# zyrlia1018/CMD-GEN

Measured on AMD Instinct MI355X. Metric: denoising steps/sec, higher is better.
Workload: dtype f32

## Files before the change

### cmdgen_amd/csrc/cmdgen_api.hip

```cpp
#include "cmdgen_host.h"
#include "cmdgen_launch.h"
#include "cmdgen_wlayout.h"

std::string g_create_error;

extern "C" const char* cmdgen_version(void) { return "cmdgen_hip 0.1 (gfx950)"; }

extern "C" const char* cmdgen_last_error(const cmdgen_handle* h) { return h ? h->err.c_str() : g_create_error.c_str(); }

extern "C" int cmdgen_create(const cmdgen_config* cfg, int device, cmdgen_handle** out) {
    if (!cfg || !out) return fail(nullptr, CMDGEN_EINVAL, "null argument");
    const int H = cfg->hidden_nf;
    if (!(H == 64 || H == 128 || H == 256 || H == 512))
        return fail(nullptr, CMDGEN_EINVAL, "hidden_nf=%d unsupported: the gfx950 kernels tile 64 columns per wave and are built for 64, 128, 256 and 512", H);
    if (cfg->inv_sublayers < 1 || cfg->inv_sublayers > 8) return fail(nullptr, CMDGEN_EINVAL, "inv_sublayers=%d out of range [1, 8]", cfg->inv_sublayers);
    if (cfg->n_layers < 1 || cfg->n_layers > CMDGEN_MAX_LAYERS) return fail(nullptr, CMDGEN_EINVAL, "n_layers out of range");
    if (cfg->phar_nf < 1 || 2 * cfg->phar_nf > CMDGEN_MAX_SMALL || cfg->residue_nf < 1 ||
        2 * cfg->residue_nf > CMDGEN_MAX_SMALL || cfg->joint_nf < 1 || cfg->joint_nf + 1 > CMDGEN_MAX_SMALL)
        return fail(nullptr, CMDGEN_EINVAL, "feature sizes exceed the small-MLP bound %d", CMDGEN_MAX_SMALL);
    if (cfg->timesteps < 1) return fail(nullptr, CMDGEN_EINVAL, "timesteps < 1");
    if (cfg->update_pocket_coords && cfg->no_com_projection)
        return fail(nullptr, CMDGEN_EINVAL, "update_pocket_coords (joint model) and no_com_projection (SimpleConditionalDDPM) are exclusive");
    int ndev = 0;
    if (hipGetDeviceCount(&ndev) != hipSuccess || device < 0 || device >= ndev)
// ... 140 lines not shown
    GET(dy + "phar_encoder.0.weight", 2 * d.P * d.P); UP(s.pe0_w); GET(dy + "phar_encoder.0.bias", 2 * d.P); UP(s.pe0_b);
    GET(dy + "phar_encoder.2.weight", d.J * 2 * d.P); UP(s.pe2_w); GET(dy + "phar_encoder.2.bias", d.J); UP(s.pe2_b);
    GET(dy + "phar_decoder.0.weight", 2 * d.P * d.J); UP(s.pd0_w); GET(dy + "phar_decoder.0.bias", 2 * d.P); UP(s.pd0_b);
    GET(dy + "phar_decoder.2.weight", d.P * 2 * d.P); UP(s.pd2_w); GET(dy + "phar_decoder.2.bias", d.P); UP(s.pd2_b);
    GET(dy + "residue_encoder.0.weight", 2 * d.R * d.R); UP(s.re0_w); GET(dy + "residue_encoder.0.bias", 2 * d.R); UP(s.re0_b);
    GET(dy + "residue_encoder.2.weight", d.J * 2 * d.R); UP(s.re2_w); GET(dy + "residue_encoder.2.bias", d.J); UP(s.re2_b);
    GET(dy + "residue_decoder.0.weight", 2 * d.R * d.J); UP(s.rd0_w); GET(dy + "residue_decoder.0.bias", 2 * d.R); UP(s.rd0_b);
    GET(dy + "residue_decoder.2.weight", d.R * 2 * d.R); UP(s.rd2_w); GET(dy + "residue_decoder.2.bias", d.R); UP(s.rd2_b);
    {
        std::vector<float> pack;
        for (const char* nm : {"phar_encoder.0.weight", "phar_encoder.0.bias", "phar_encoder.2.weight", "phar_encoder.2.bias",
                               "residue_encoder.0.weight", "residue_encoder.0.bias", "residue_encoder.2.weight", "residue_encoder.2.bias"}) {
            auto it = h->staged.find(dy + nm);
            if (it == h->staged.end()) return fail(h, CMDGEN_ESTATE, "missing tensor '%s%s'", dy.c_str(), nm);
            pack.insert(pack.end(), it->second.begin(), it->second.end());
        }
        rc = upload(h, pack, &s.enc_pack); if (rc) return rc;
    }
    {
        GET(dy + "egnn.embedding.weight", H * d.dyn);
        std::vector<float> t((size_t)H * d.dyn);
        for (int c = 0; c < H; ++c) for (int k = 0; k < d.dyn; ++k) t[(size_t)k * H + c] = (*v)[(size_t)c * d.dyn + k];
        rc = upload(h, t, &s.emb_wT); if (rc) return rc;
        GET(dy + "egnn.embedding.bias", H); UP(s.emb_b);
    }
    {
        GET(dy + "egnn.embedding_out.weight", d.dyn * H);
        std::vector<float> t((size_t)H * d.dyn);
        for (int j = 0; j < d.dyn; ++j) for (int k = 0; k < H; ++k) t[(size_t)k * d.dyn + j] = (*v)[(size_t)j * H + k];
        rc = upload(h, t, &s.embo_wT); if (rc) return rc;
        GET(dy + "egnn.embedding_out.bias", d.dyn); UP(s.embo_b);
    }
    const int nfeat = d.sin ? 24 : 2;
    const int ld1 = 2 * H + nfeat;
    for (int b = 0; b < d.L; ++b)
    for (int sub = 0; sub < d.S; ++sub) {
        LayerW lw{};
        const std::string g = dy + "egnn.e_block_" + std::to_string(b) + ".gcl_" + std::to_string(sub) + ".";
        const std::string c = dy + "egnn.e_block_" + std::to_string(b) + ".gcl_equiv.";
        auto split_first = [&](const std::string& wname, const std::string& bname, WPack* Wpq,
                               const float** bias, const float** wr, const float** wd, const float** we) -> int {
            const std::vector<float>* w; int r = get_w(h, wname, (size_t)H * ld1, &w); if (r) return r;
            std::vector<float> AB((size_t)2 * H * H);
            std::vector<float> vr(H), vd(H);
            for (int o = 0; o < H; ++o) {
                for (int k = 0; k < H; ++k) {
// ... 41 lines not shown
#undef GET
#undef UP
    h->layers = std::move(layers);
    h->finalized = true;
    h->user_coef_K = -1;
    release_chains(h);
    if (h->have_layout) replan(h);
    return CMDGEN_OK;
}

static inline size_t edge_lds_bytes(int max_n) { return (size_t)max_n * (sizeof(float4) + 3 * sizeof(int)); }
static const size_t kEdgeLdsMax = 156 * 1024;

PlanInput plan_input(const cmdgen_handle* h) {
    PlanInput in;
    const Dims& d = h->dims;
    in.H = d.H; in.L = d.L; in.S = d.S; in.joint = d.joint != 0; in.sin = d.sin != 0; in.cutoff = d.cutoff2 >= 0.f;
    in.n_cus = h->n_cus; in.gemm_split = h->gemm_split;
    in.B = (int)h->cur_nphar.size(); in.nph = h->cur_nphar.data(); in.npk = h->cur_npocket.data();
    in.N = h->lay.N; in.Nl = h->lay.Nl; in.max_n = h->lay.max_n;
    in.opts = &h->opts;
    if (!h->layers.empty()) {
        in.W2 = in.W7 = in.Wpq_e = PlanPacks::of_uploaded(d.H); in.W3 = PlanPacks::of_uploaded(2 * d.H);
    }
    return in;
}
void replan(cmdgen_handle* h) { h->plan = make_plan(plan_input(h)); }

static int set_layout_impl(cmdgen_handle* h, int64_t batch, const int64_t* nph, const int64_t* npk, bool on_stream, hipStream_t stream);
extern "C" int cmdgen_set_layout(cmdgen_handle* h, int64_t batch, const int64_t* nph, const int64_t* npk) {
    return set_layout_impl(h, batch, nph, npk, false, nullptr);
}
extern "C" int cmdgen_set_layout_on_stream(cmdgen_handle* h, int64_t batch, const int64_t* nph, const int64_t* npk, cmdgen_stream stream) {
    return set_layout_impl(h, batch, nph, npk, true, (hipStream_t)stream);
}
static int set_layout_impl(cmdgen_handle* h, int64_t batch, const int64_t* nph, const int64_t* npk, bool on_stream, hipStream_t stream) {
    if (!h || batch < 1 || !nph || !npk) return fail(h, CMDGEN_EINVAL, "bad layout arguments");
    if (h->have_layout && (int64_t)h->cur_nphar.size() == batch &&
        memcmp(h->cur_nphar.data(), nph, batch * sizeof(int64_t)) == 0 &&
        memcmp(h->cur_npocket.data(), npk, batch * sizeof(int64_t)) == 0)
        return CMDGEN_OK;
    ++h->eval_gen;
    hipSetDevice(h->device);
    const Dims& d = h->dims;
    const int B = (int)batch;
    std::vector<int> vph(B), vpk(B), bph(B), bpk(B);
// ... 117 lines not shown
    if (!h) return CMDGEN_EINVAL;
    if (!h->have_layout) return fail(h, CMDGEN_ESTATE, "no batch layout (cmdgen_set_layout)");
    hipSetDevice(h->device);
    h->last_stream = s;
    if (h->agg_dirty) {
        HIPCHK(h, hipMemsetAsync(h->work.agg, 0, (size_t)h->lay.N * h->dims.H * sizeof(float), s));
        h->agg_dirty = false;
    }
    return 0;
}

EvalLaunch make_launch(cmdgen_handle* h) {
    EvalLaunch a; a.lay = h->lay; a.w = h->work; a.d = h->dims; a.sw = h->small; a.layers = h->layers.data();
    a.plan = h->plan;
    a.prof_events = nullptr; a.ablate = 0;
    if (!a.plan.node64 && !a.plan.dead_skip) a.w.need_qc = nullptr;
    a.w.hop_levels = a.plan.dead_skip >= 2 ? h->dims.L : 1;
    if (!a.plan.dead_skip) a.w.ehop = nullptr;
    return a;
}

static const char* const kOptionKeys[] = {
    "node_mt", "edge_mt", "coord_mt", "embed_mt", "edge_wgs_per_cu", "coord_wgs_per_cu", "e128_wgs_per_cu", "e128_fused", "half_engine", "edge_fullk", "node64", "node16_split", "node16w",
    "proj_in_coord", "dead_skip", "write_embed", "graph_steps",
    "wgrad_split", "wgrad_tile", "wgrad_split_wgs128", "wgrad_split_wgs64", "wgrad_wgs", "dgrad_mt", "dgrad_tail", "wgrad_stream", "train_half", "wgrad_silu", "train_node16", "wgrad_k128"};

static void drop_graphs(cmdgen_handle* h) {
    hipSetDevice(h->device);
    if (h->own_stream) hipStreamSynchronize(h->own_stream);
    if (h->have_layout) hipStreamSynchronize(h->last_stream);
    drop_chain_graphs(h);
}
static void refresh_tune(cmdgen_handle* h) {
    TrainTune t;
    t.wgrad_split = (int)opt_of(h, "wgrad_split", t.wgrad_split); t.wgrad_tile = (int)opt_of(h, "wgrad_tile", t.wgrad_tile);
    t.wgrad_split_wgs128 = (int)opt_of(h, "wgrad_split_wgs128", t.wgrad_split_wgs128); t.wgrad_split_wgs64 = (int)opt_of(h, "wgrad_split_wgs64", t.wgrad_split_wgs64);
    t.wgrad_wgs = (int)opt_of(h, "wgrad_wgs", t.wgrad_wgs); t.dgrad_mt = (int)opt_of(h, "dgrad_mt", t.dgrad_mt); t.dgrad_tail = (int)opt_of(h, "dgrad_tail", t.dgrad_tail);
    t.wgrad_stream = (int)opt_of(h, "wgrad_stream", t.wgrad_stream); t.wgrad_k128 = (int)opt_of(h, "wgrad_k128", t.wgrad_k128);
    h->tune = t;
}

extern "C" int cmdgen_set_option(cmdgen_handle* h, const char* key, int64_t value, int32_t unset) {
    if (!h || !key) return fail(h, CMDGEN_EINVAL, "null argument");
    bool known = false;
    for (const char* k : kOptionKeys) known = known || strcmp(k, key) == 0;
    if (!known) return fail(h, CMDGEN_EINVAL, "unknown option '%s'", key);
    drop_graphs(h);
// ... 891 lines not shown
```

### cmdgen_amd/csrc/cmdgen_dev.h

```cpp
#pragma once
#include <hip/hip_runtime.h>
#include <stdint.h>
#include <vector>
#include "cmdgen_split.h"
#include "cmdgen_plan.h"

typedef float f32x16 __attribute__((ext_vector_type(16)));

#define CMDGEN_MAX_LAYERS 16
#define CMDGEN_MAX_SMALL 64

struct WPack {
    const float4* w32;
    const float4* w16;
    const void*   ws;
    const void*   ws16;
    const void*   wh;
    const void*   wh16;
    float         wh_scale;
    float         wh_inv;
    const float*  wh_dev;
};

struct LayerW {
// ... 8 lines not shown
    const float*  ba;
    WPack W3;
    const float*  b3;
    WPack W4;
    const float*  b4;
    WPack Wpq_c;
    const float*  b6;
    const float*  wr_c;
    const float*  wd_c;
    const float*  we_c;
    WPack W7;
    const float*  b7;
    const float*  w5;
};

struct SmallW {
    const float *pe0_w, *pe0_b, *pe2_w, *pe2_b;
    const float *pd0_w, *pd0_b, *pd2_w, *pd2_b;
    const float *re0_w, *re0_b, *re2_w, *re2_b;
    const float *rd0_w, *rd0_b, *rd2_w, *rd2_b;
    const float *emb_wT, *emb_b;
    const float *embo_wT, *embo_b;
    const float *enc_pack;
};

struct Dims {
    int P, R, J, H, L;
    int dyn;
    int attention, use_tanh, condition_time;
    int no_com;
    int joint;
    float cutoff2;
    float norm_constant, norm_factor, coords_range;
    int S;
    int sin;
    float sin_freq[6];
    int agg_mean;
    float norm_x, norm_h, bias_h;
};

struct Layout {
    int B, Nl, Np, N;
    int Nm;
    int max_n;
    const int* num_phar;
    const int* num_pocket;
    const int* phar_base;
// ... 406 lines not shown
```

### cmdgen_amd/csrc/cmdgen_plan.h

```cpp
#pragma once
#include <cstdint>
#include <cstring>
#include <map>
#include <string>

enum class PlanEngine { fp32, bf3, half };
inline int plan_mfmas_per_product(PlanEngine e) { return e == PlanEngine::fp32 ? 1 : e == PlanEngine::bf3 ? 6 : 3; }

enum class MsgKernel { tiles, fullk32, e128 };
enum class NodeKernel { tiles, node16w, node32p, node64, node64e, node64d };
enum class CoordKernel { tiles, fullk32, fullk32_proj, e128 };

struct PlanPacks {
    bool ws = false, wh = false, ws16 = false, wh16 = false;
    static PlanPacks of_uploaded(int in) { return PlanPacks{true, true, in % 128 == 0, in % 128 == 0}; }
};

struct PlanInput {
    int H = 256, L = 1, S = 1;
    bool joint = false, sin = false, cutoff = true;
    int n_cus = 256;
    bool gemm_split = true;
    int B = 0;
    const int64_t* nph = nullptr; const int64_t* npk = nullptr;
    int N = 0, Nl = 0, max_n = 0;
    const std::map<std::string, int64_t>* opts = nullptr;
    PlanPacks W2, W3, W7, Wpq_e;
    bool training = false;
    int E = 0, Ec = 0;

    int64_t opt(const char* key, int64_t dflt) const { if (!opts) return dflt; auto it = opts->find(key); return it == opts->end() ? dflt : it->second; }
    bool opt_set(const char* key) const { return opts && opts->find(key) != opts->end(); }
};

struct LaunchPlan {
    MsgKernel msg = MsgKernel::tiles; NodeKernel node = NodeKernel::tiles; CoordKernel coord = CoordKernel::tiles;
    PlanEngine msg_eng = PlanEngine::fp32, node_eng = PlanEngine::fp32, coord_eng = PlanEngine::fp32;
    int node_mt = 64, edge_mt = 64, coord_mt = 64;
    int embed_mt = 16;
    int edge_grid = 512, coord_grid = 256, e128_grid = 512;
    int e128_fused = 3;
    int dead_skip = 0, write_embed = 1;
    int gemm_split = 1, half_engine = 0, node16_split = 0, node64 = 0, node16w = 1, edge_fullk = 0, proj_in_coord = 0;
    bool fwd_half = false, node_half = false;
    bool reads_frag = false;
};

inline LaunchPlan make_plan(const PlanInput& in) {
    LaunchPlan p;
    const int n_cus = in.n_cus, H = in.H;
    const bool split = in.gemm_split, sp256 = H == 256 && split;
    const int he_opt = (int)in.opt("half_engine", 1);
    const bool half_opt = he_opt == 2 || (he_opt == 1 && in.cutoff);
    const bool half = sp256 && half_opt;
    p.gemm_split = split ? 1 : 0;
    p.half_engine = split && half_opt ? 1 : 0;

    double e_est = 0.0, ec_est = 0.0;
    const int64_t N = (int64_t)in.N;
    for (int b = 0; b < in.B; ++b) {
        const double n = (double)(in.nph[b] + in.npk[b]);
        const bool full = !in.cutoff;
        const double deg = full ? n : (n <= 128.0 ? 9.0 : 36.0);
        const double dnode = deg < n ? deg : n;
        double dphar = full ? n : 0.6 * (double)in.nph[b] + (n <= 128.0 ? 0.15 : 0.13) * (double)in.npk[b];
        if (dphar > n) dphar = n;
// ... 45 lines not shown
    {
        int on = 0;
        if (sp256 && n_cus > 0) {
            const int ncu = n_cus, t64 = (in.N + 63) / 64, t32 = (in.N + 31) / 32;
            const float cost64 = (float)((t64 + ncu - 1) / ncu);
            const int full = t32 / (2 * ncu), rem = t32 - full * 2 * ncu;
            float cost32 = 1.12f * full + (rem == 0 ? 0.f : rem <= ncu ? 0.62f : 1.12f);
            if (half) cost32 = 1.9f * full + (rem == 0 ? 0.f : rem <= ncu ? 1.22f : 1.9f);
            on = cost64 < cost32 && !(half && node_mt == 16);
            if (half && node_mt != 16) on = 32;
            if (on == 32 && t32 > ncu && t64 <= ncu) on = 8;
            else if (on == 32 && t64 > ncu) on = 2;
            if (in.opt_set("node64")) { const int64_t v = in.opt("node64", 0); on = v == 32 ? 32 : v == 8 ? 8 : v == 2 ? 2 : v != 0; }
        }
        p.node64 = on;
        p.dead_skip = (in.joint || in.S != 1) ? 0 : (int)in.opt("dead_skip", 2);
    }
    p.node16_split = (split && H >= 128 && in.opt("node16_split", 1) != 0) ? 1 : 0;
    p.node16w = in.opt("node16w", 1) != 0 ? 1 : 0;
    {
        p.embed_mt = (int)in.opt("embed_mt", (((double)in.Nl / 16.0 <= 2.0 * n_cus && !in.joint) ? 16 : node_mt));
        if (p.embed_mt != 16 && p.embed_mt != 32 && p.embed_mt != 64) p.embed_mt = node_mt;
    }
    if (split && node_mt == 64 && !in.opt_set("node_mt")) node_mt = 32;
    p.node_mt = node_mt; p.edge_mt = edge_mt; p.coord_mt = coord_mt;

    const PlanEngine tiles32 = split ? PlanEngine::bf3 : PlanEngine::fp32;
    if (in.training) {
        const int train_half = (int)in.opt("train_half", 1);
        p.fwd_half = sp256 && half_opt && p.edge_fullk && in.W2.wh && train_half != 0;
        if (p.fwd_half && in.opt("train_node16", 1) != 0) p.node_mt = 16;
        p.node_half = p.fwd_half && p.node_mt == 16 && in.W3.wh16 && train_half != 2;
        p.dead_skip = 0; p.node64 = 0; p.proj_in_coord = 0;
        auto rows = [&](int n) { return n / 64 >= 4 * n_cus ? 64 : (n / 32 >= n_cus / 4 ? 32 : 16); };
        auto grid = [&](int n, int mt) { const int cap = (mt >= 64 ? 2 : 4) * n_cus, g = (int)((n / mt + 1) * 1.25) + 8; return g < n_cus / 4 ? n_cus / 4 : (g > cap ? cap : g); };
        if (!in.opt_set("edge_mt") || p.edge_mt == 128) { p.edge_mt = rows(in.E); p.edge_grid = grid(in.E, p.edge_mt); }
        if (!in.opt_set("coord_mt") || p.coord_mt == 128) { p.coord_mt = rows(in.Ec); p.coord_grid = grid(in.Ec, p.coord_mt); }
        if (p.fwd_half) {
            p.edge_mt = 32; p.edge_grid = grid(in.E, 32); p.coord_mt = 32; p.coord_grid = grid(in.Ec, 32);
        }
        const PlanEngine save32 = split && H == 256 && in.W2.ws ? PlanEngine::bf3 : PlanEngine::fp32;
        p.msg = p.fwd_half ? MsgKernel::fullk32 : MsgKernel::tiles;
        p.msg_eng = p.fwd_half ? PlanEngine::half : (p.edge_mt >= 32 ? save32 : PlanEngine::fp32);
        p.coord = p.fwd_half ? CoordKernel::fullk32 : CoordKernel::tiles;
        p.coord_eng = p.fwd_half ? PlanEngine::half : (p.coord_mt >= 32 ? save32 : PlanEngine::fp32);
        p.node = p.node_half && H == 256 ? NodeKernel::node16w : NodeKernel::tiles;
// ... 11 lines not shown
        p.node = p.node64 == 2 && eight ? NodeKernel::node64d : p.node64 == 8 && eight ? NodeKernel::node64e : p.node64 == 32 ? NodeKernel::node32p : NodeKernel::node64;
    } else if (H == 256 && node_mt == 16 && p.node16_split && p.node16w && in.W3.ws16) {
        p.node = NodeKernel::node16w; p.node_eng = half && in.W3.wh16 ? PlanEngine::half : PlanEngine::bf3;
    } else {
        p.node = NodeKernel::tiles;
        p.node_eng = node_mt >= 32 ? tiles32 : (p.node16_split && in.W3.ws16 ? PlanEngine::bf3 : PlanEngine::fp32);
    }
    if (coord_mt == 128 && in.W7.ws) { p.coord = CoordKernel::e128; p.coord_eng = half && in.W7.wh ? PlanEngine::half : PlanEngine::bf3; }
    else if (p.edge_fullk && coord_mt == 32) { p.coord = CoordKernel::fullk32; p.coord_eng = half && in.W7.wh ? PlanEngine::half : PlanEngine::bf3; }
    else { p.coord = CoordKernel::tiles; p.coord_eng = coord_mt >= 32 ? tiles32 : PlanEngine::fp32; }
    p.reads_frag = p.msg == MsgKernel::tiles || p.coord == CoordKernel::tiles || p.node == NodeKernel::tiles;
    const bool can = p.node == NodeKernel::node16w && p.coord == CoordKernel::fullk32 && in.S == 1 && in.L > 1 && !in.joint && p.node_eng == p.coord_eng &&
                     (p.node_eng == PlanEngine::half ? in.Wpq_e.wh16 : in.Wpq_e.ws16);
    p.proj_in_coord = can && in.opt("proj_in_coord", 1) != 0 ? 1 : 0;
    if (p.proj_in_coord) p.coord = CoordKernel::fullk32_proj;
    return p;
}

inline bool plan_query(const LaunchPlan& p, const char* key, int64_t* value) {
    const struct { const char* key; int64_t v; } keys[] = {
        {"node_mt", p.node_mt}, {"edge_mt", p.edge_mt}, {"coord_mt", p.coord_mt}, {"edge_grid", p.edge_grid}, {"coord_grid", p.coord_grid},
        {"e128_fused", p.e128_fused}, {"gemm_split", p.gemm_split}, {"half_engine", p.half_engine}, {"node16_split", p.node16_split},
        {"node64", p.node64}, {"node16w", p.node16w}, {"proj_in_coord", p.proj_in_coord}, {"edge_fullk", p.edge_fullk}, {"dead_skip", p.dead_skip},
        {"msg_mfmas_per_product", plan_mfmas_per_product(p.msg_eng)}, {"node_mfmas_per_product", plan_mfmas_per_product(p.node_eng)},
        {"coord_mfmas_per_product", plan_mfmas_per_product(p.coord_eng)}};
    for (const auto& k : keys) if (strcmp(k.key, key) == 0) { *value = k.v; return true; }
    return false;
}
```

### cmdgen_amd/csrc/kernels_egnn_graph.hip

```cpp
#ifndef CMDGEN_H_PART
#define CMDGEN_H_PART 0
#endif
#include "cmdgen_egnn_common.h"

__device__ __forceinline__ int flat_node(int i, int nl, int pb, int qb, int Nl) {
    return i < nl ? pb + i : Nl + qb + (i - nl);
}

#if CMDGEN_H_PART == 0
__global__ void k_edge_count(Layout lay, Work w, Dims d, const float* __restrict__ xh_phar,
                             const float* __restrict__ xh_pocket) {
    extern __shared__ float4 spos[];
    int* sdeg = reinterpret_cast<int*>(spos + lay.max_n);
    const int b = blockIdx.x, tid = threadIdx.x;
    const int nl = lay.num_phar[b], np = lay.num_pocket[b], n = nl + np;
    const int pb = lay.phar_base[b], qb = lay.pocket_base[b];
    const int ldp = 3 + d.P, ldq = 3 + d.R;
    for (int i = tid; i < n; i += blockDim.x) {
        float4 p;
        if (i < nl) {
            const float* s = xh_phar + (size_t)(pb + i) * ldp;
            p = make_float4(s[0], s[1], s[2], 0.f);
            w.X0[pb + i] = p;
            for (int l = 0; l < d.L; ++l) w.ACC[(size_t)l * lay.Nm + pb + i] = make_float4(0.f, 0.f, 0.f, 0.f);
// ... 186 lines not shown
                for (int e = lane; e < dg; e += 64) w.ehop[off + e] = lvl;
            }
        }
    }
    if (b == 0 && tid == 0) *w.nan_flag = 0;
    if (b == lay.B - 1 && tid == 0) {
        const int E = s_base[1] + (w.pocketE[b] - eph_b);
        const int Ec = d.joint ? s_base[4] + w.pocketEnsQ[b] : s_base[3] + w.pocketEns[b];
        w.totals[0] = E; w.totals[1] = Ec;
        atomicAdd(&w.counters[1], (unsigned long long)E);
        atomicAdd(&w.counters[2], (unsigned long long)Ec);
    }
}
#if CMDGEN_H_PART == 0
__global__ void k_edge_write(Layout lay, Work w, Dims d) { edge_write_body(lay, w, d, blockIdx.x); }
#endif

template <int H, int MT, bool SP>
__device__ __forceinline__ void embed_body(const Layout& lay, const Work& w, const Dims& d, const SmallW& sw, const LayerW& lw0,
                                           const float* __restrict__ xh_phar,
                                           const float* __restrict__ xh_pocket,
                                           const float* __restrict__ t_arr,
                                           const float4* __restrict__ coef, const ChainState* chain, const TrainSave& sv,
                                           const PocketCache& pc, const int blk, const int part = 2) {
    if (pc.c != nullptr && blk * MT >= lay.Nl) {
        const int row0 = blk * MT, nvalid = min(MT, lay.N - row0);
        const float t = coef[chain->step].w;
        constexpr int LPR = H / 4;
        const int c4 = threadIdx.x % LPR, rsub = threadIdx.x / LPR;
        const float4 dh = reinterpret_cast<const float4*>(pc.dh)[c4], dP = reinterpret_cast<const float4*>(pc.dP)[c4],
                     dQ = reinterpret_cast<const float4*>(pc.dQ)[c4];
        auto axpy = [&](const float4& a, const float4& b) { return make_float4(fmaf(t, b.x, a.x), fmaf(t, b.y, a.y), fmaf(t, b.z, a.z), fmaf(t, b.w, a.w)); };
#pragma unroll 4
        for (int r = rsub; r < nvalid; r += 4) {
            const size_t q = (size_t)(row0 + r - lay.Nl) * LPR + c4, o = (size_t)(row0 + r) * LPR + c4;
            reinterpret_cast<float4*>(w.h)[o] = axpy(reinterpret_cast<const float4*>(pc.c)[q], dh);
            reinterpret_cast<float4*>(w.P)[o] = axpy(reinterpret_cast<const float4*>(pc.P0)[q], dP);
            reinterpret_cast<float4*>(w.Q)[o] = axpy(reinterpret_cast<const float4*>(pc.Q0)[q], dQ);
        }
        return;
    }
#if CMDGEN_STAMPS == 3
    unsigned long long est_[8] = {0,0,0,0,0,0,0,0}, est_t = __builtin_amdgcn_s_memtime(); const unsigned long long est_b = est_t;
#define ESTAMP(i) do { const unsigned long long n_ = __builtin_amdgcn_s_memtime(); est_[i] += n_ - est_t; est_t = n_; } while (0)
#else
#define ESTAMP(i) do {} while (0)
#endif
    __shared__ __attribute__((aligned(16))) float buf[MT * LDA(H)];
    __shared__ float s_in[MT][CMDGEN_MAX_SMALL];
    __shared__ float s_h1[MT][CMDGEN_MAX_SMALL];
    __shared__ float s_h2[MT][CMDGEN_MAX_SMALL + 1];
    const int tid = threadIdx.x, nthr = H;
    const int row0 = blk * MT;
    const int nvalid = min(MT, lay.N - row0);
    const int ldp = 3 + d.P, ldq = 3 + d.R;
    const int Fmax = max(d.P, d.R), F1max = 2 * Fmax;
    typedef Eng<MT, SP> G;
    typename G::Carry carry;
    const typename G::Frag f0 = G::frag(lw0.Wpq_e, H / 8, 0, (part == 1 ? H / 64 : 0) + (tid >> 6));
    G::prefetch(f0, carry);
    const ColVec<MT> b1v = col_load<MT>(lw0.b1, tid >> 6);
    const float t_chain = t_arr ? 0.f : coef[chain->step].w;
    extern __shared__ float s_enc[];
    const int seg_n[8] = {2 * d.P * d.P, 2 * d.P, d.J * 2 * d.P, d.J, 2 * d.R * d.R, 2 * d.R, d.J * 2 * d.R, d.J};
    const float* const seg_p[8] = {sw.pe0_w, sw.pe0_b, sw.pe2_w, sw.pe2_b, sw.re0_w, sw.re0_b, sw.re2_w, sw.re2_b};
    int seg_o[9];
    seg_o[0] = 0;
#pragma unroll
    for (int q = 0; q < 8; ++q) seg_o[q + 1] = seg_o[q] + seg_n[q];
    constexpr int NIN = (MT * CMDGEN_MAX_SMALL + H - 1) / H;
    float vin[NIN];
#pragma unroll
    for (int q = 0; q < NIN; ++q) {
        const int idx = tid + q * nthr;
        vin[q] = 0.f;
        if (idx < MT * Fmax) {
            const int r = idx / Fmax, k = idx - r * Fmax, n = row0 + r;
            if (r < nvalid) {
                if (n < lay.Nl) { if (k < d.P) vin[q] = xh_phar[(size_t)n * ldp + 3 + k]; }
                else if (k < d.R) vin[q] = xh_pocket[(size_t)(n - lay.Nl) * ldq + 3 + k];
            }
        }
    }
    if (sw.enc_pack) {
        for (int i = tid; i < seg_o[8]; i += nthr) s_enc[i] = sw.enc_pack[i];
    } else
    for (int base = 0; base < seg_o[8]; base += 16 * nthr) {
        float v[16];
#pragma unroll
        for (int q = 0; q < 16; ++q) {
            const int gi = base + q * nthr + tid;
            v[q] = 0.f;
            if (gi < seg_o[8]) {
                int sg = 0;
#pragma unroll
                for (int u = 1; u < 8; ++u) sg += gi >= seg_o[u];
                v[q] = seg_p[sg][gi - seg_o[sg]];
            }
        }
#pragma unroll
        for (int q = 0; q < 16; ++q) {
            const int gi = base + q * nthr + tid;
            if (gi < seg_o[8]) s_enc[gi] = v[q];
        }
    }
    const float *pe0w = s_enc + seg_o[0], *pe0b = s_enc + seg_o[1], *pe2w = s_enc + seg_o[2], *pe2b = s_enc + seg_o[3];
    const float *re0w = s_enc + seg_o[4], *re0b = s_enc + seg_o[5], *re2w = s_enc + seg_o[6], *re2b = s_enc + seg_o[7];
#pragma unroll
    for (int q = 0; q < NIN; ++q) {
        const int idx = tid + q * nthr;
        if (idx < MT * Fmax) { const int r = idx / Fmax; s_in[r][idx - r * Fmax] = vin[q]; }
    }
    lds_barrier();
    ESTAMP(0);
    for (int idx = tid; idx < MT * F1max; idx += nthr) {
        const int r = idx / F1max, o = idx - r * F1max;
        const int n = row0 + r;
        if (r >= nvalid) continue;
        const bool ph = n < lay.Nl;
        const int F = ph ? d.P : d.R;
        if (o >= 2 * F) continue;
        const float* W = (ph ? pe0w : re0w) + o * F;
        float s = (ph ? pe0b : re0b)[o];
#pragma unroll 4
        for (int k = 0; k < F; ++k) s = fmaf(s_in[r][k], W[k], s);
        const float act = silu_f(s);
        s_h1[r][o] = act;
        if (sv.enc1_l) {
            if (ph) { sv.enc1_l[(size_t)n * 2 * F + o] = s; sv.enca_l[(size_t)n * 2 * F + o] = act; }
            else { sv.enc1_p[(size_t)(n - lay.Nl) * 2 * F + o] = s; sv.enca_p[(size_t)(n - lay.Nl) * 2 * F + o] = act; }
        }
    }
    lds_barrier();
    ESTAMP(1);
    for (int idx = tid; idx < MT * d.dyn; idx += nthr) {
        const int r = idx / d.dyn, j = idx - r * d.dyn;
        const int n = row0 + r;
        float s = 0.f;
        if (r < nvalid) {
            if (j < d.J) {
                const bool ph = n < lay.Nl;
                const int F2 = 2 * (ph ? d.P : d.R);
                const float* W = (ph ? pe2w : re2w) + j * F2;
                s = (ph ? pe2b : re2b)[j];
#pragma unroll 4
                for (int k = 0; k < F2; ++k) s = fmaf(s_h1[r][k], W[k], s);
            } else {
                s = t_arr ? t_arr[lay.node_sample[n]] : t_chain;
            }
            if (sv.hdyn) sv.hdyn[(size_t)n * d.dyn + j] = s;
        }
        s_h2[r][j] = s;
    }
    lds_barrier();
    ESTAMP(2);
    {
        const int c = tid;
        const float bc = sw.emb_b[c];
        float accr[MT];
#pragma unroll
        for (int r = 0; r < MT; ++r) accr[r] = bc;
        for (int k0 = 0; k0 < d.dyn; k0 += 16) {
            float wk[16];
#pragma unroll
            for (int j = 0; j < 16; ++j) wk[j] = k0 + j < d.dyn ? sw.emb_wT[(size_t)(k0 + j) * H + c] : 0.f;
#pragma unroll
            for (int j = 0; j < 16; ++j)
                if (k0 + j < d.dyn) {
#pragma unroll
                    for (int r = 0; r < MT; ++r) accr[r] = fmaf(s_h2[r][k0 + j], wk[j], accr[r]);
                }
        }
#pragma unroll
        for (int r = 0; r < MT; ++r) {
            const float s = r < nvalid ? accr[r] : 0.f;
            buf[r * LDA(H) + c] = s;
            if (r < nvalid && part != 1) {
                w.h[(size_t)(row0 + r) * H + c] = s;
                if (sv.h) sv.h[(size_t)(row0 + r) * H + c] = s;
            }
        }
    }
    lds_barrier();
    ESTAMP(3);
    tile_project_pq<H, MT, SP>(buf, lw0.Wpq_e, b1v, w.P, w.Q, row0, nvalid, part != 1, carry, f0, part != 0);
    ESTAMP(4);
#if CMDGEN_STAMPS == 3
    if ((threadIdx.x & 63) == 0) { const int wv = threadIdx.x >> 6; for (int i = 0; i < 5; ++i) atomicAdd(&w.dbg[wv * 8 + i], est_[i]);
        atomicAdd(&w.dbg[32 + wv], __builtin_amdgcn_s_memtime() - est_b); atomicAdd(&w.dbg[40], 1ull); }
#endif
#undef ESTAMP
}
template <int H, int MT, bool SP>
__global__ __launch_bounds__(H) void k_embed(Layout lay, Work w, Dims d, SmallW sw, LayerW lw0, const float* __restrict__ xh_phar,
                                             const float* __restrict__ xh_pocket, const float* __restrict__ t_arr,
                                             const float4* __restrict__ coef, const ChainState* chain, TrainSave sv, PocketCache pc) {
    embed_body<H, MT, SP>(lay, w, d, sw, lw0, xh_phar, xh_pocket, t_arr, coef, chain, sv, pc, (int)blockIdx.x);
}
template <int MT, bool SP>
__global__ __launch_bounds__(256) void k_write_embed(Layout lay, Work w, Dims d, SmallW sw, LayerW lw0, const float* __restrict__ xh_phar,
                                                     const float* __restrict__ xh_pocket, const float* __restrict__ t_arr,
                                                     const float4* __restrict__ coef, const ChainState* chain, PocketCache pc, int npair) {
    const int i = (int)blockIdx.x - lay.B;
    if (i < 0) edge_write_body(lay, w, d, (int)blockIdx.x);
    else if (i < 2 * npair) embed_body<256, MT, SP>(lay, w, d, sw, lw0, xh_phar, xh_pocket, t_arr, coef, chain, TrainSave{}, pc, i >> 1, i & 1);
    else embed_body<256, MT, SP>(lay, w, d, sw, lw0, xh_phar, xh_pocket, t_arr, coef, chain, TrainSave{}, pc, i - npair, 2);
}

template <int H, int MT, bool SP> static void launch_embed(const EvalLaunch& a, const float* xp, const float* xq, const float* t,
                                                  const float4* coef, ChainState* chain, hipStream_t s) {
    if constexpr (H == 512 && MT == 64) launch_embed<H, 32, SP>(a, xp, xq, t, coef, chain, s);
    else {
        const int nt = (a.lay.N + MT - 1) / MT;
        const Dims& d = a.d;
        const size_t shm = sizeof(float) * (size_t)(2 * d.P * d.P + 2 * d.P + d.J * 2 * d.P + d.J + 2 * d.R * d.R + 2 * d.R + d.J * 2 * d.R + d.J);
        if (a.save) hipLaunchKernelGGL((k_embed<H, MT, false>), dim3(nt), dim3(H), shm, s, a.lay, a.w, a.d, a.sw, a.layers[0], xp, xq, t, coef,
                                       (const ChainState*)chain, *a.save, PocketCache{});
        else hipLaunchKernelGGL((k_embed<H, MT, SP>), dim3(nt), dim3(H), shm, s, a.lay, a.w, a.d, a.sw, a.layers[0], xp, xq, t, coef,
                                (const ChainState*)chain, TrainSave{}, (chain && !t) ? a.pcache : PocketCache{});
    }
}
template <int H, int MT, bool SP> static void launch_write_embed(const EvalLaunch& a, const float* xp, const float* xq, const float* t,
                                                                 const float4* coef, ChainState* chain, hipStream_t s) {
    if constexpr (H == 256) {
        const int nt = (a.lay.N + MT - 1) / MT;
        const Dims& d = a.d;
        const size_t shm_e = sizeof(float) * (size_t)(2 * d.P * d.P + 2 * d.P + d.J * 2 * d.P + d.J + 2 * d.R * d.R + 2 * d.R + d.J * 2 * d.R + d.J);
        const size_t shm_w = (size_t)a.lay.max_n * (sizeof(float4) + 3 * sizeof(int));
        const PocketCache pc = (chain && !t) ? a.pcache : PocketCache{};
        const int npair = pc.c ? (a.lay.Nl + MT - 1) / MT : 0;
        hipLaunchKernelGGL((k_write_embed<MT, SP>), dim3(a.lay.B + nt + npair), dim3(256), shm_e > shm_w ? shm_e : shm_w, s, a.lay, a.w, a.d, a.sw,
                           a.layers[0], xp, xq, t, coef, (const ChainState*)chain, pc, npair);
    }
}
template <int H> static void embed_only_H(const EvalLaunch& a, const float* xp, const float* xq, const float* t, hipStream_t s) {
    MT_DISPATCH(a.plan.node_mt, a.plan.gemm_split != 0, launch_embed, a, xp, xq, t, nullptr, nullptr, s);
}
template <int H> static void embed_tiles_H(const EvalLaunch& a, int mt, const float* xp, const float* xq, const float* t, const float4* coef, ChainState* chain, hipStream_t s) {
    MT_DISPATCH(mt, a.plan.gemm_split != 0, launch_embed, a, xp, xq, t, coef, chain, s);
}
#if CMDGEN_H_PART == 0
void cmdgen_launch_embed_tiles(const EvalLaunch& a, int mt, const float* xp, const float* xq, const float* t, const float4* coef, ChainState* chain, hipStream_t s) {
    if (a.d.H == 256) embed_tiles_H<256>(a, mt, xp, xq, t, coef, chain, s); else cmdgen_launch_embed_tiles_hx(a, mt, xp, xq, t, coef, chain, s);
}
#else
void cmdgen_launch_embed_tiles_hx(const EvalLaunch& a, int mt, const float* xp, const float* xq, const float* t, const float4* coef, ChainState* chain, hipStream_t s) {
    switch (a.d.H) {
        case 512: embed_tiles_H<512>(a, mt, xp, xq, t, coef, chain, s); break;
        case 128: embed_tiles_H<128>(a, mt, xp, xq, t, coef, chain, s); break;
        case 64:  embed_tiles_H<64>(a, mt, xp, xq, t, coef, chain, s); break;
        default: break;
    }
}
#endif
#if CMDGEN_H_PART == 0
// ... 58 lines not shown
```

Baseline: 187,900.

## Add MFMA path for ligand embedding encoder and input projection at H=256

Adds a specialised embedding path for full 16-row ligand tiles at H=256 that runs the second phar-encoder layer and the embedding linear on MFMA instructions. It uses weights prepacked on the host into lane-fragment layout, replacing the scalar FMA loops and the per-block staging of encoder weights in shared memory. The path is gated by a new plan option that defaults on only when the ligand count is large enough and the embed tile size is 16. It adds code complexity and register use in the embed kernel.

```diff
diff --git a/cmdgen_amd/csrc/cmdgen_api.hip b/cmdgen_amd/csrc/cmdgen_api.hip
--- a/cmdgen_amd/csrc/cmdgen_api.hip
+++ b/cmdgen_amd/csrc/cmdgen_api.hip
@@ -186,6 +186,21 @@
         std::vector<float> t((size_t)H * d.dyn);
         for (int c = 0; c < H; ++c) for (int k = 0; k < d.dyn; ++k) t[(size_t)k * H + c] = (*v)[(size_t)c * d.dyn + k];
         rc = upload(h, t, &s.emb_wT); if (rc) return rc;
+        s.emf_pack = nullptr;
+        if (d.P == EMF_P && d.J == EMF_J && d.dyn == EMF_J + 1) {
+            const std::vector<float>* we = v;
+            GET(dy + "phar_encoder.2.weight", d.J * 2 * d.P);
+            const std::vector<float>* w2 = v;
+            std::vector<float> pack((size_t)EMF_J * 2 * EMF_P + (size_t)(H / 16) * 64 * EMF_KE_LD, 0.f);
+            for (int nt = 0; nt < EMF_J / 16; ++nt) for (int lane = 0; lane < 64; ++lane) for (int st = 0; st < 2 * EMF_P / 4; ++st)
+                pack[(size_t)(nt * 64 + lane) * (2 * EMF_P / 4) + st] = (*w2)[(size_t)(16 * nt + lane % 16) * 2 * EMF_P + 4 * st + lane / 16];
+            float* pe = pack.data() + EMF_J * 2 * EMF_P;
+            for (int nt = 0; nt < H / 16; ++nt) for (int lane = 0; lane < 64; ++lane) for (int st = 0; st < EMF_KE; ++st) {
+                const int k = 4 * st + lane / 16;
+                pe[(size_t)(nt * 64 + lane) * EMF_KE_LD + st] = k < d.dyn ? (*we)[(size_t)(16 * nt + lane % 16) * d.dyn + k] : 0.f;
+            }
+            rc = upload(h, pack, &s.emf_pack); if (rc) return rc;
+        }
         GET(dy + "egnn.embedding.bias", H); UP(s.emb_b);
     }
     {
@@ -273,6 +288,7 @@
     in.opts = &h->opts;
     if (!h->layers.empty()) {
         in.W2 = in.W7 = in.Wpq_e = PlanPacks::of_uploaded(d.H); in.W3 = PlanPacks::of_uploaded(2 * d.H);
+        in.embed_pack = h->small.emf_pack != nullptr;
     }
     return in;
 }
@@ -436,7 +452,7 @@
 
 static const char* const kOptionKeys[] = {
     "node_mt", "edge_mt", "coord_mt", "embed_mt", "edge_wgs_per_cu", "coord_wgs_per_cu", "e128_wgs_per_cu", "e128_fused", "half_engine", "edge_fullk", "node64", "node16_split", "node16w",
-    "proj_in_coord", "dead_skip", "write_embed", "graph_steps",
+    "proj_in_coord", "embed_mfma", "dead_skip", "write_embed", "graph_steps",
     "wgrad_split", "wgrad_tile", "wgrad_split_wgs128", "wgrad_split_wgs64", "wgrad_wgs", "dgrad_mt", "dgrad_tail", "wgrad_stream", "train_half", "wgrad_silu", "train_node16", "wgrad_k128"};
 
 static void drop_graphs(cmdgen_handle* h) {
diff --git a/cmdgen_amd/csrc/cmdgen_dev.h b/cmdgen_amd/csrc/cmdgen_dev.h
--- a/cmdgen_amd/csrc/cmdgen_dev.h
+++ b/cmdgen_amd/csrc/cmdgen_dev.h
@@ -54,7 +54,12 @@
     const float *emb_wT, *emb_b;
     const float *embo_wT, *embo_b;
     const float *enc_pack;
-};
+    const float *emf_pack;
+};
+#define EMF_P 8
+#define EMF_J 32
+#define EMF_KE 9
+#define EMF_KE_LD 12
 
 struct Dims {
     int P, R, J, H, L;
diff --git a/cmdgen_amd/csrc/cmdgen_plan.h b/cmdgen_amd/csrc/cmdgen_plan.h
--- a/cmdgen_amd/csrc/cmdgen_plan.h
+++ b/cmdgen_amd/csrc/cmdgen_plan.h
@@ -28,6 +28,7 @@
     PlanPacks W2, W3, W7, Wpq_e;
     bool training = false;
     int E = 0, Ec = 0;
+    bool embed_pack = false;
 
     int64_t opt(const char* key, int64_t dflt) const { if (!opts) return dflt; auto it = opts->find(key); return it == opts->end() ? dflt : it->second; }
     bool opt_set(const char* key) const { return opts && opts->find(key) != opts->end(); }
@@ -42,6 +43,7 @@
     int e128_fused = 3;
     int dead_skip = 0, write_embed = 1;
     int gemm_split = 1, half_engine = 0, node16_split = 0, node64 = 0, node16w = 1, edge_fullk = 0, proj_in_coord = 0;
+    int embed_mfma = 0;
     bool fwd_half = false, node_half = false;
     bool reads_frag = false;
 };
@@ -133,6 +135,7 @@
         p.embed_mt = (int)in.opt("embed_mt", (((double)in.Nl / 16.0 <= 2.0 * n_cus && !in.joint) ? 16 : node_mt));
         if (p.embed_mt != 16 && p.embed_mt != 32 && p.embed_mt != 64) p.embed_mt = node_mt;
     }
+    p.embed_mfma = H == 256 && in.embed_pack && !in.training && (p.embed_mt == 16 || node_mt == 16) && in.opt("embed_mfma", in.Nl >= 30 * 16 ? 1 : 0) != 0 ? 1 : 0;
     if (split && node_mt == 64 && !in.opt_set("node_mt")) node_mt = 32;
     p.node_mt = node_mt; p.edge_mt = edge_mt; p.coord_mt = coord_mt;
 
@@ -190,6 +193,7 @@
         {"node_mt", p.node_mt}, {"edge_mt", p.edge_mt}, {"coord_mt", p.coord_mt}, {"edge_grid", p.edge_grid}, {"coord_grid", p.coord_grid},
         {"e128_fused", p.e128_fused}, {"gemm_split", p.gemm_split}, {"half_engine", p.half_engine}, {"node16_split", p.node16_split},
         {"node64", p.node64}, {"node16w", p.node16w}, {"proj_in_coord", p.proj_in_coord}, {"edge_fullk", p.edge_fullk}, {"dead_skip", p.dead_skip},
+        {"embed_mfma", p.embed_mfma},
         {"msg_mfmas_per_product", plan_mfmas_per_product(p.msg_eng)}, {"node_mfmas_per_product", plan_mfmas_per_product(p.node_eng)},
         {"coord_mfmas_per_product", plan_mfmas_per_product(p.coord_eng)}};
     for (const auto& k : keys) if (strcmp(k.key, key) == 0) { *value = k.v; return true; }
diff --git a/cmdgen_amd/csrc/kernels_egnn_graph.hip b/cmdgen_amd/csrc/kernels_egnn_graph.hip
--- a/cmdgen_amd/csrc/kernels_egnn_graph.hip
+++ b/cmdgen_amd/csrc/kernels_egnn_graph.hip
@@ -232,7 +232,7 @@
                                            const float* __restrict__ xh_pocket,
                                            const float* __restrict__ t_arr,
                                            const float4* __restrict__ coef, const ChainState* chain, const TrainSave& sv,
-                                           const PocketCache& pc, const int blk, const int part = 2) {
+                                           const PocketCache& pc, const int blk, const int part = 2, const int emf = 0) {
     if (pc.c != nullptr && blk * MT >= lay.Nl) {
         const int row0 = blk * MT, nvalid = min(MT, lay.N - row0);
         const float t = coef[chain->step].w;
@@ -271,128 +271,205 @@
     G::prefetch(f0, carry);
     const ColVec<MT> b1v = col_load<MT>(lw0.b1, tid >> 6);
     const float t_chain = t_arr ? 0.f : coef[chain->step].w;
-    extern __shared__ float s_enc[];
-    const int seg_n[8] = {2 * d.P * d.P, 2 * d.P, d.J * 2 * d.P, d.J, 2 * d.R * d.R, 2 * d.R, d.J * 2 * d.R, d.J};
-    const float* const seg_p[8] = {sw.pe0_w, sw.pe0_b, sw.pe2_w, sw.pe2_b, sw.re0_w, sw.re0_b, sw.re2_w, sw.re2_b};
-    int seg_o[9];
-    seg_o[0] = 0;
-#pragma unroll
-    for (int q = 0; q < 8; ++q) seg_o[q + 1] = seg_o[q] + seg_n[q];
-    constexpr int NIN = (MT * CMDGEN_MAX_SMALL + H - 1) / H;
-    float vin[NIN];
-#pragma unroll
-    for (int q = 0; q < NIN; ++q) {
-        const int idx = tid + q * nthr;
-        vin[q] = 0.f;
-        if (idx < MT * Fmax) {
-            const int r = idx / Fmax, k = idx - r * Fmax, n = row0 + r;
+    bool mf = false;
+    if constexpr (H == 256 && MT == 16) mf = emf != 0 && row0 + MT <= lay.Nl;
+    if (mf) {
+        if constexpr (H == 256 && MT == 16) {
+            const int lane = tid & 63, wv = tid >> 6, l16 = lane & 15, g = lane >> 4;
+            const int r0 = tid >> 4, o0 = tid & 15;
+            const float4 w0a = reinterpret_cast<const float4*>(sw.pe0_w)[2 * o0], w0b = reinterpret_cast<const float4*>(sw.pe0_w)[2 * o0 + 1];
+            const float b0 = sw.pe0_b[o0];
+            float xin[EMF_P];
+#pragma unroll
+            for (int k = 0; k < EMF_P; ++k) xin[k] = xh_phar[(size_t)(row0 + r0) * ldp + 3 + k];
+            float4 w2 = make_float4(0.f, 0.f, 0.f, 0.f);
+            float b2 = 0.f, tcol = 0.f;
+            if (wv < 2) { w2 = reinterpret_cast<const float4*>(sw.emf_pack)[wv * 64 + lane]; b2 = sw.pe2_b[16 * wv + l16]; }
+            else if (wv == 2 && lane < MT) tcol = t_arr ? t_arr[lay.node_sample[row0 + lane]] : t_chain;
+            const float4* pe = reinterpret_cast<const float4*>(sw.emf_pack + EMF_J * 2 * EMF_P) + (size_t)(4 * wv * 64 + lane) * (EMF_KE_LD / 4);
+            float we[4][EMF_KE_LD], be[4];
+#pragma unroll
+            for (int i = 0; i < 4; ++i) {
+#pragma unroll
+                for (int q = 0; q < EMF_KE_LD / 4; ++q) {
+                    const float4 v = pe[(size_t)i * 64 * (EMF_KE_LD / 4) + q];
+                    we[i][4 * q] = v.x; we[i][4 * q + 1] = v.y; we[i][4 * q + 2] = v.z; we[i][4 * q + 3] = v.w;
+                }
+                be[i] = sw.emb_b[16 * (4 * wv + i) + l16];
+            }
+            ESTAMP(0);
+            {
+                const float w0[EMF_P] = {w0a.x, w0a.y, w0a.z, w0a.w, w0b.x, w0b.y, w0b.z, w0b.w};
+                float s = b0;
+#pragma unroll
+                for (int k = 0; k < EMF_P; ++k) s = fmaf(xin[k], w0[k], s);
+                buf[r0 * LDA(H) + o0] = silu_f(s);
+            }
+            lds_barrier();
+            ESTAMP(1);
+            if (wv < 2) {
+                const float w2v[4] = {w2.x, w2.y, w2.z, w2.w};
+                f32x4v c = {b2, b2, b2, b2};
+#pragma unroll
+                for (int st = 0; st < 2 * EMF_P / 4; ++st) CMDGEN_MFMA16(c, buf[l16 * LDA(H) + 4 * st + g], w2v[st]);
+#pragma unroll
+                for (int v = 0; v < 4; ++v) s_h2[4 * g + v][16 * wv + l16] = c[v];
+            } else if (wv == 2 && lane < MT) {
+                s_h2[lane][EMF_J] = tcol;
+#pragma unroll
+                for (int k = EMF_J + 1; k < 4 * EMF_KE; ++k) s_h2[lane][k] = 0.f;
+            }
+            lds_barrier();
+            ESTAMP(2);
+            {
+                float a[EMF_KE];
+#pragma unroll
+                for (int st = 0; st < EMF_KE; ++st) a[st] = s_h2[l16][4 * st + g];
+                f32x4v c[4];
+#pragma unroll
+                for (int i = 0; i < 4; ++i) c[i] = f32x4v{be[i], be[i], be[i], be[i]};
+#pragma unroll
+                for (int st = 0; st < EMF_KE; ++st) {
+#pragma unroll
+                    for (int i = 0; i < 4; ++i) CMDGEN_MFMA16(c[i], a[st], we[i][st]);
+                }
+#pragma unroll
+                for (int i = 0; i < 4; ++i) {
+#pragma unroll
+                    for (int v = 0; v < 4; ++v) {
+                        const int r = 4 * g + v, col = 16 * (4 * wv + i) + l16;
+                        buf[r * LDA(H) + col] = c[i][v];
+                        if (part != 1) w.h[(size_t)(row0 + r) * H + col] = c[i][v];
+                    }
+                }
+            }
+            lds_barrier();
+            ESTAMP(3);
+        }
+    } else {
+        extern __shared__ float s_enc[];
+        const int seg_n[8] = {2 * d.P * d.P, 2 * d.P, d.J * 2 * d.P, d.J, 2 * d.R * d.R, 2 * d.R, d.J * 2 * d.R, d.J};
+        const float* const seg_p[8] = {sw.pe0_w, sw.pe0_b, sw.pe2_w, sw.pe2_b, sw.re0_w, sw.re0_b, sw.re2_w, sw.re2_b};
+        int seg_o[9];
+        seg_o[0] = 0;
+#pragma unroll
+        for (int q = 0; q < 8; ++q) seg_o[q + 1] = seg_o[q] + seg_n[q];
+        constexpr int NIN = (MT * CMDGEN_MAX_SMALL + H - 1) / H;
+        float vin[NIN];
+#pragma unroll
+        for (int q = 0; q < NIN; ++q) {
+            const int idx = tid + q * nthr;
+            vin[q] = 0.f;
+            if (idx < MT * Fmax) {
+                const int r = idx / Fmax, k = idx - r * Fmax, n = row0 + r;
+                if (r < nvalid) {
+                    if (n < lay.Nl) { if (k < d.P) vin[q] = xh_phar[(size_t)n * ldp + 3 + k]; }
+                    else if (k < d.R) vin[q] = xh_pocket[(size_t)(n - lay.Nl) * ldq + 3 + k];
+                }
+            }
+        }
+        if (sw.enc_pack) {
+            for (int i = tid; i < seg_o[8]; i += nthr) s_enc[i] = sw.enc_pack[i];
+        } else
+        for (int base = 0; base < seg_o[8]; base += 16 * nthr) {
+            float v[16];
+#pragma unroll
+            for (int q = 0; q < 16; ++q) {
+                const int gi = base + q * nthr + tid;
+                v[q] = 0.f;
+                if (gi < seg_o[8]) {
+                    int sg = 0;
+#pragma unroll
+                    for (int u = 1; u < 8; ++u) sg += gi >= seg_o[u];
+                    v[q] = seg_p[sg][gi - seg_o[sg]];
+                }
+            }
+#pragma unroll
+            for (int q = 0; q < 16; ++q) {
+                const int gi = base + q * nthr + tid;
+                if (gi < seg_o[8]) s_enc[gi] = v[q];
+            }
+        }
+        const float *pe0w = s_enc + seg_o[0], *pe0b = s_enc + seg_o[1], *pe2w = s_enc + seg_o[2], *pe2b = s_enc + seg_o[3];
+        const float *re0w = s_enc + seg_o[4], *re0b = s_enc + seg_o[5], *re2w = s_enc + seg_o[6], *re2b = s_enc + seg_o[7];
+#pragma unroll
+        for (int q = 0; q < NIN; ++q) {
+            const int idx = tid + q * nthr;
+            if (idx < MT * Fmax) { const int r = idx / Fmax; s_in[r][idx - r * Fmax] = vin[q]; }
+        }
+        lds_barrier();
+        ESTAMP(0);
+        for (int idx = tid; idx < MT * F1max; idx += nthr) {
+            const int r = idx / F1max, o = idx - r * F1max;
+            const int n = row0 + r;
+            if (r >= nvalid) continue;
+            const bool ph = n < lay.Nl;
+            const int F = ph ? d.P : d.R;
+            if (o >= 2 * F) continue;
+            const float* W = (ph ? pe0w : re0w) + o * F;
+            float s = (ph ? pe0b : re0b)[o];
+#pragma unroll 4
+            for (int k = 0; k < F; ++k) s = fmaf(s_in[r][k], W[k], s);
+            const float act = silu_f(s);
+            s_h1[r][o] = act;
+            if (sv.enc1_l) {
+                if (ph) { sv.enc1_l[(size_t)n * 2 * F + o] = s; sv.enca_l[(size_t)n * 2 * F + o] = act; }
+                else { sv.enc1_p[(size_t)(n - lay.Nl) * 2 * F + o] = s; sv.enca_p[(size_t)(n - lay.Nl) * 2 * F + o] = act; }
+            }
+        }
+        lds_barrier();
+        ESTAMP(1);
+        for (int idx = tid; idx < MT * d.dyn; idx += nthr) {
+            const int r = idx / d.dyn, j = idx - r * d.dyn;
+            const int n = row0 + r;
+            float s = 0.f;
             if (r < nvalid) {
-                if (n < lay.Nl) { if (k < d.P) vin[q] = xh_phar[(size_t)n * ldp + 3 + k]; }
-                else if (k < d.R) vin[q] = xh_pocket[(size_t)(n - lay.Nl) * ldq + 3 + k];
-            }
-        }
-    }
-    if (sw.enc_pack) {
-        for (int i = tid; i < seg_o[8]; i += nthr) s_enc[i] = sw.enc_pack[i];
-    } else
-    for (int base = 0; base < seg_o[8]; base += 16 * nthr) {
-        float v[16];
-#pragma unroll
-        for (int q = 0; q < 16; ++q) {
-            const int gi = base + q * nthr + tid;
-            v[q] = 0.f;
-            if (gi < seg_o[8]) {
-                int sg = 0;
-#pragma unroll
-                for (int u = 1; u < 8; ++u) sg += gi >= seg_o[u];
-                v[q] = seg_p[sg][gi - seg_o[sg]];
-            }
-        }
-#pragma unroll
-        for (int q = 0; q < 16; ++q) {
-            const int gi = base + q * nthr + tid;
-            if (gi < seg_o[8]) s_enc[gi] = v[q];
-        }
-    }
-    const float *pe0w = s_enc + seg_o[0], *pe0b = s_enc + seg_o[1], *pe2w = s_enc + seg_o[2], *pe2b = s_enc + seg_o[3];
-    const float *re0w = s_enc + seg_o[4], *re0b = s_enc + seg_o[5], *re2w = s_enc + seg_o[6], *re2b = s_enc + seg_o[7];
-#pragma unroll
-    for (int q = 0; q < NIN; ++q) {
-        const int idx = tid + q * nthr;
-        if (idx < MT * Fmax) { const int r = idx / Fmax; s_in[r][idx - r * Fmax] = vin[q]; }
-    }
-    lds_barrier();
-    ESTAMP(0);
-    for (int idx = tid; idx < MT * F1max; idx += nthr) {
-        const int r = idx / F1max, o = idx - r * F1max;
-        const int n = row0 + r;
-        if (r >= nvalid) continue;
-        const bool ph = n < lay.Nl;
-        const int F = ph ? d.P : d.R;
-        if (o >= 2 * F) continue;
-        const float* W = (ph ? pe0w : re0w) + o * F;
-        float s = (ph ? pe0b : re0b)[o];
+                if (j < d.J) {
+                    const bool ph = n < lay.Nl;
+                    const int F2 = 2 * (ph ? d.P : d.R);
+                    const float* W = (ph ? pe2w : re2w) + j * F2;
+                    s = (ph ? pe2b : re2b)[j];
 #pragma unroll 4
-        for (int k = 0; k < F; ++k) s = fmaf(s_in[r][k], W[k], s);
-        const float act = silu_f(s);
-        s_h1[r][o] = act;
-        if (sv.enc1_l) {
-            if (ph) { sv.enc1_l[(size_t)n * 2 * F + o] = s; sv.enca_l[(size_t)n * 2 * F + o] = act; }
-            else { sv.enc1_p[(size_t)(n - lay.Nl) * 2 * F + o] = s; sv.enca_p[(size_t)(n - lay.Nl) * 2 * F + o] = act; }
-        }
-    }
-    lds_barrier();
-    ESTAMP(1);
-    for (int idx = tid; idx < MT * d.dyn; idx += nthr) {
-        const int r = idx / d.dyn, j = idx - r * d.dyn;
-        const int n = row0 + r;
-        float s = 0.f;
-        if (r < nvalid) {
-            if (j < d.J) {
-                const bool ph = n < lay.Nl;
-                const int F2 = 2 * (ph ? d.P : d.R);
-                const float* W = (ph ? pe2w : re2w) + j * F2;
-                s = (ph ? pe2b : re2b)[j];
-#pragma unroll 4
-                for (int k = 0; k < F2; ++k) s = fmaf(s_h1[r][k], W[k], s);
-            } else {
-                s = t_arr ? t_arr[lay.node_sample[n]] : t_chain;
-            }
-            if (sv.hdyn) sv.hdyn[(size_t)n * d.dyn + j] = s;
-        }
-        s_h2[r][j] = s;
-    }
-    lds_barrier();
-    ESTAMP(2);
-    {
-        const int c = tid;
-        const float bc = sw.emb_b[c];
-        float accr[MT];
-#pragma unroll
-        for (int r = 0; r < MT; ++r) accr[r] = bc;
-        for (int k0 = 0; k0 < d.dyn; k0 += 16) {
-            float wk[16];
-#pragma unroll
-            for (int j = 0; j < 16; ++j) wk[j] = k0 + j < d.dyn ? sw.emb_wT[(size_t)(k0 + j) * H + c] : 0.f;
-#pragma unroll
-            for (int j = 0; j < 16; ++j)
-                if (k0 + j < d.dyn) {
-#pragma unroll
-                    for (int r = 0; r < MT; ++r) accr[r] = fmaf(s_h2[r][k0 + j], wk[j], accr[r]);
-                }
-        }
-#pragma unroll
-        for (int r = 0; r < MT; ++r) {
-            const float s = r < nvalid ? accr[r] : 0.f;
-            buf[r * LDA(H) + c] = s;
-            if (r < nvalid && part != 1) {
-                w.h[(size_t)(row0 + r) * H + c] = s;
-                if (sv.h) sv.h[(size_t)(row0 + r) * H + c] = s;
-            }
-        }
-    }
-    lds_barrier();
-    ESTAMP(3);
+                    for (int k = 0; k < F2; ++k) s = fmaf(s_h1[r][k], W[k], s);
+                } else {
+                    s = t_arr ? t_arr[lay.node_sample[n]] : t_chain;
+                }
+                if (sv.hdyn) sv.hdyn[(size_t)n * d.dyn + j] = s;
+            }
+            s_h2[r][j] = s;
+        }
+        lds_barrier();
+        ESTAMP(2);
+        {
+            const int c = tid;
+            const float bc = sw.emb_b[c];
+            float accr[MT];
+#pragma unroll
+            for (int r = 0; r < MT; ++r) accr[r] = bc;
+            for (int k0 = 0; k0 < d.dyn; k0 += 16) {
+                float wk[16];
+#pragma unroll
+                for (int j = 0; j < 16; ++j) wk[j] = k0 + j < d.dyn ? sw.emb_wT[(size_t)(k0 + j) * H + c] : 0.f;
+#pragma unroll
+                for (int j = 0; j < 16; ++j)
+                    if (k0 + j < d.dyn) {
+#pragma unroll
+                        for (int r = 0; r < MT; ++r) accr[r] = fmaf(s_h2[r][k0 + j], wk[j], accr[r]);
+                    }
+            }
+#pragma unroll
+            for (int r = 0; r < MT; ++r) {
+                const float s = r < nvalid ? accr[r] : 0.f;
+                buf[r * LDA(H) + c] = s;
+                if (r < nvalid && part != 1) {
+                    w.h[(size_t)(row0 + r) * H + c] = s;
+                    if (sv.h) sv.h[(size_t)(row0 + r) * H + c] = s;
+                }
+            }
+        }
+        lds_barrier();
+        ESTAMP(3);
+    }
     tile_project_pq<H, MT, SP>(buf, lw0.Wpq_e, b1v, w.P, w.Q, row0, nvalid, part != 1, carry, f0, part != 0);
     ESTAMP(4);
 #if CMDGEN_STAMPS == 3
@@ -404,19 +481,20 @@
 template <int H, int MT, bool SP>
 __global__ __launch_bounds__(H) void k_embed(Layout lay, Work w, Dims d, SmallW sw, LayerW lw0, const float* __restrict__ xh_phar,
                                              const float* __restrict__ xh_pocket, const float* __restrict__ t_arr,
-                                             const float4* __restrict__ coef, const ChainState* chain, TrainSave sv, PocketCache pc) {
-    embed_body<H, MT, SP>(lay, w, d, sw, lw0, xh_phar, xh_pocket, t_arr, coef, chain, sv, pc, (int)blockIdx.x);
+                                             const float4* __restrict__ coef, const ChainState* chain, TrainSave sv, PocketCache pc, int emf) {
+    embed_body<H, MT, SP>(lay, w, d, sw, lw0, xh_phar, xh_pocket, t_arr, coef, chain, sv, pc, (int)blockIdx.x, 2, emf);
 }
 template <int MT, bool SP>
 __global__ __launch_bounds__(256) void k_write_embed(Layout lay, Work w, Dims d, SmallW sw, LayerW lw0, const float* __restrict__ xh_phar,
                                                      const float* __restrict__ xh_pocket, const float* __restrict__ t_arr,
-                                                     const float4* __restrict__ coef, const ChainState* chain, PocketCache pc, int npair) {
+                                                     const float4* __restrict__ coef, const ChainState* chain, PocketCache pc, int npair, int emf) {
     const int i = (int)blockIdx.x - lay.B;
     if (i < 0) edge_write_body(lay, w, d, (int)blockIdx.x);
-    else if (i < 2 * npair) embed_body<256, MT, SP>(lay, w, d, sw, lw0, xh_phar, xh_pocket, t_arr, coef, chain, TrainSave{}, pc, i >> 1, i & 1);
-    else embed_body<256, MT, SP>(lay, w, d, sw, lw0, xh_phar, xh_pocket, t_arr, coef, chain, TrainSave{}, pc, i - npair, 2);
-}
-
+    else if (i < 2 * npair) embed_body<256, MT, SP>(lay, w, d, sw, lw0, xh_phar, xh_pocket, t_arr, coef, chain, TrainSave{}, pc, i >> 1, i & 1, emf);
+    else embed_body<256, MT, SP>(lay, w, d, sw, lw0, xh_phar, xh_pocket, t_arr, coef, chain, TrainSave{}, pc, i - npair, 2, emf);
+}
+
+static inline int embed_mfma_arg(const EvalLaunch& a) { return a.plan.embed_mfma && a.sw.emf_pack && !a.save ? 1 : 0; }
 template <int H, int MT, bool SP> static void launch_embed(const EvalLaunch& a, const float* xp, const float* xq, const float* t,
                                                   const float4* coef, ChainState* chain, hipStream_t s) {
     if constexpr (H == 512 && MT == 64) launch_embed<H, 32, SP>(a, xp, xq, t, coef, chain, s);
@@ -425,9 +503,9 @@
         const Dims& d = a.d;
         const size_t shm = sizeof(float) * (size_t)(2 * d.P * d.P + 2 * d.P + d.J * 2 * d.P + d.J + 2 * d.R * d.R + 2 * d.R + d.J * 2 * d.R + d.J);
         if (a.save) hipLaunchKernelGGL((k_embed<H, MT, false>), dim3(nt), dim3(H), shm, s, a.lay, a.w, a.d, a.sw, a.layers[0], xp, xq, t, coef,
-                                       (const ChainState*)chain, *a.save, PocketCache{});
+                                       (const ChainState*)chain, *a.save, PocketCache{}, 0);
         else hipLaunchKernelGGL((k_embed<H, MT, SP>), dim3(nt), dim3(H), shm, s, a.lay, a.w, a.d, a.sw, a.layers[0], xp, xq, t, coef,
-                                (const ChainState*)chain, TrainSave{}, (chain && !t) ? a.pcache : PocketCache{});
+                                (const ChainState*)chain, TrainSave{}, (chain && !t) ? a.pcache : PocketCache{}, embed_mfma_arg(a));
     }
 }
 template <int H, int MT, bool SP> static void launch_write_embed(const EvalLaunch& a, const float* xp, const float* xq, const float* t,
@@ -440,7 +518,7 @@
         const PocketCache pc = (chain && !t) ? a.pcache : PocketCache{};
         const int npair = pc.c ? (a.lay.Nl + MT - 1) / MT : 0;
         hipLaunchKernelGGL((k_write_embed<MT, SP>), dim3(a.lay.B + nt + npair), dim3(256), shm_e > shm_w ? shm_e : shm_w, s, a.lay, a.w, a.d, a.sw,
-                           a.layers[0], xp, xq, t, coef, (const ChainState*)chain, pc, npair);
+                           a.layers[0], xp, xq, t, coef, (const ChainState*)chain, pc, npair, embed_mfma_arg(a));
     }
 }
 template <int H> static void embed_only_H(const EvalLaunch& a, const float* xp, const float* xq, const float* t, hipStream_t s) {
```

New measurement: 190,000, median of 6. 1.1% higher.
